# maxrmorrison/torbi

Hardware: AMD Instinct MI355X
Metric: timesteps decoded/sec, 1440 states batch=512 (higher is better)
Workload: dtype f32; 1 GPU; 1440 states, 500 frames, batch=512 per GPU, fp32, dense transition (BASELINE configs[2]); decode = forward + argmax + backtrace, inputs resident in HBM; parallelism=single GPU, streams=2

## Files before the change

### torbi_amd/csrc/lazy_backtrace.hpp

```cpp
#pragma once

#include <hip/hip_runtime.h>
#include <stdint.h>
#include <math.h>

#include "wave_reduce.hpp"

namespace lazy {

constexpr int kSentinel = 0x7fffffff;

__device__ __forceinline__ void take_better(float &v, int &i, float ov, int oi) {
    if (ov > v || (ov == v && oi < i)) { v = ov; i = oi; }
}

__device__ __forceinline__ int wave_first_argmax(float v, int i) {
#pragma unroll
    for (int off = 32; off > 0; off >>= 1) {
        const float ov = __shfl_xor(v, off, 64);
        const int oi = __shfl_xor(i, off, 64);
        take_better(v, i, ov, oi);
    }
    return i;
}

__device__ __forceinline__ void scan1(float c, int i, float &best, int &arg) {
    if (c > best) { best = c; arg = i; }
    else if (arg == kSentinel) { best = c; arg = i; }
}

template <int VEC>
__device__ __forceinline__ void backtrace_item(const float *__restrict__ h, const float *__restrict__ trans, int f,
                                               int32_t *__restrict__ o, int T, int S, int lane) {
    f = f < 1 ? 1 : (f > T ? T : f);

    float best = -INFINITY;
    int arg = kSentinel;
    {
        const float *row = h + (size_t)(f - 1) * S;
        if (VEC == 4) {
            for (int i = 4 * lane; i < S; i += 256) {
                const float4 v = *reinterpret_cast<const float4 *>(row + i);
                scan1(v.x, i, best, arg); scan1(v.y, i + 1, best, arg);
                scan1(v.z, i + 2, best, arg); scan1(v.w, i + 3, best, arg);
            }
        } else {
            for (int i = lane; i < S; i += 64) scan1(row[i], i, best, arg);
        }
    }
    int j = wave_first_argmax(best, arg);

    for (int tt = f - 1 + lane; tt < T; tt += 64) o[tt] = j;

    for (int tt = f - 1; tt >= 1; --tt) {
        const float *row = h + (size_t)(tt - 1) * S;
        const float *tr = trans + (size_t)j * S;
        best = -INFINITY;
        arg = kSentinel;
        if (VEC == 4) {
            for (int i = 4 * lane; i < S; i += 256) {
                const float4 p = *reinterpret_cast<const float4 *>(row + i);
                const float4 q = *reinterpret_cast<const float4 *>(tr + i);
                scan1(p.x + q.x, i, best, arg); scan1(p.y + q.y, i + 1, best, arg);
                scan1(p.z + q.z, i + 2, best, arg); scan1(p.w + q.w, i + 3, best, arg);
            }
        } else {
            for (int i = lane; i < S; i += 64) scan1(row[i] + tr[i], i, best, arg);
        }
        j = wave_first_argmax(best, arg);
        if (lane == 0) o[tt - 1] = j;
    }
}

template <int VEC>
__global__ __launch_bounds__(64) void backtrace_kernel(const float *__restrict__ hist,
                                                       const float *__restrict__ trans,
                                                       const int32_t *__restrict__ frames,
                                                       int32_t *__restrict__ out, int B, int T, int S) {
    const int b = blockIdx.x;
    backtrace_item<VEC>(hist + (size_t)b * T * S, trans, frames[b], out + (size_t)b * T, T, S, threadIdx.x);
}

template <int NQ>
__device__ __forceinline__ int lane_first_equal(const float4 (&v)[NQ], float m, int lane, int S) {
    int k = kSentinel;
#pragma unroll
    for (int q = NQ - 1; q >= 0; --q) {
        const int i = 4 * lane + 256 * q;
        if (i < S) {
            int kq = v[q].w == m ? i + 3 : kSentinel;
            kq = v[q].z == m ? i + 2 : kq;
            kq = v[q].y == m ? i + 1 : kq;
            kq = v[q].x == m ? i : kq;
            k = min(k, kq);
        }
    }
    return k;
}

template <int NQ>
__device__ __forceinline__ float lane_max(const float4 (&v)[NQ], int lane, int S) {
    float m = -INFINITY;
#pragma unroll
    for (int q = 0; q < NQ; ++q)
        if (4 * lane + 256 * q < S)
            m = __builtin_fmaxf(__builtin_fmaxf(m, __builtin_fmaxf(v[q].x, v[q].y)), __builtin_fmaxf(v[q].z, v[q].w));
    return m;
}

template <int NQ>
__device__ __forceinline__ int wave_first_argmax4(const float4 (&v)[NQ], int lane, int S) {
    const float m = wavered::wave_reduce_f32(lane_max<NQ>(v, lane, S), wavered::MaxOp());
    const int k = wavered::wave_min_i32(lane_first_equal<NQ>(v, m, lane, S));
    return k < S ? k : 0;
}

template <int NQ>
__device__ __forceinline__ void backtrace_prefetch_item(const float *__restrict__ h, const float *__restrict__ trans,
                                                        int f, int32_t *__restrict__ o, int T, int S, int lane) {
    f = f < 1 ? 1 : (f > T ? T : f);
    const float4 zero = make_float4(0.f, 0.f, 0.f, 0.f);

    float4 cur[NQ], nxt[NQ];
    {
        const float *row = h + (size_t)(f - 1) * S;
#pragma unroll
        for (int q = 0; q < NQ; ++q) {
            const int i = 4 * lane + 256 * q;
            cur[q] = i < S ? *reinterpret_cast<const float4 *>(row + i) : zero;
        }
    }
    {
        const float *row = h + (size_t)(f >= 2 ? f - 2 : 0) * S;
#pragma unroll
        for (int q = 0; q < NQ; ++q) {
            const int i = 4 * lane + 256 * q;
            nxt[q] = i < S ? *reinterpret_cast<const float4 *>(row + i) : zero;
        }
    }
    int j = wave_first_argmax4<NQ>(cur, lane, S);
    for (int tt = f - 1 + lane; tt < T; tt += 64) o[tt] = j;

    for (int tt = f - 1; tt >= 1; --tt) {
        const float *tr = trans + (size_t)j * S;
        float4 q4[NQ];
#pragma unroll
        for (int q = 0; q < NQ; ++q) {
            const int i = 4 * lane + 256 * q;
            q4[q] = i < S ? *reinterpret_cast<const float4 *>(tr + i) : zero;
        }
#pragma unroll
        for (int q = 0; q < NQ; ++q) cur[q] = nxt[q];
        {
            const float *row = h + (size_t)(tt >= 2 ? tt - 2 : 0) * S;
#pragma unroll
            for (int q = 0; q < NQ; ++q) {
                const int i = 4 * lane + 256 * q;
                nxt[q] = i < S ? *reinterpret_cast<const float4 *>(row + i) : zero;
            }
        }
        float4 cand[NQ];
#pragma unroll
        for (int q = 0; q < NQ; ++q)
            cand[q] = make_float4(cur[q].x + q4[q].x, cur[q].y + q4[q].y, cur[q].z + q4[q].z, cur[q].w + q4[q].w);
        j = wave_first_argmax4<NQ>(cand, lane, S);
        if (lane == 0) o[tt - 1] = j;
    }
}

template <int NQ>
__global__ __launch_bounds__(64) void backtrace_prefetch_kernel(const float *__restrict__ hist,
                                                                const float *__restrict__ trans,
                                                                const int32_t *__restrict__ frames,
                                                                int32_t *__restrict__ out, int B, int T, int S,
                                                                const int32_t *__restrict__ narrow) {
    if (narrow && *narrow <= 512) return;
    const int b = blockIdx.x;
    backtrace_prefetch_item<NQ>(hist + (size_t)b * T * S, trans, frames[b], out + (size_t)b * T, T, S, threadIdx.x);
}

template <int NQ>
struct GatherWalker {
    const float *__restrict__ h;
    const float *__restrict__ rowmax;
    const float2 *__restrict__ sorted;
    int SpP, shift, S, lane;
    __device__ __forceinline__ int first_state(int t) const {
        const float4 zero = make_float4(0.f, 0.f, 0.f, 0.f);
        float4 last[NQ];
        const float *row = h + (size_t)t * S;
#pragma unroll
        for (int q = 0; q < NQ; ++q) {
            const int i = 4 * lane + 256 * q;
            last[q] = i < S ? *reinterpret_cast<const float4 *>(row + i) : zero;
        }
        return wave_first_argmax4<NQ>(last, lane, S);
    }
    __device__ __forceinline__ int step(int j, int tt) const {
        const int Sp = (S + 15) / 16 * 16;
        const float2 *row = sorted + (size_t)j * SpP;
        float2 ent = row[lane];
        const float hmax = rowmax[tt - 1];
        const float *hrow = h + (size_t)(tt - 1) * S;
        float bv = -INFINITY;
        int bi = kSentinel;
        float best = -INFINITY;
        for (int k0 = 0; k0 < Sp; k0 += 64) {
            const int kn = k0 + 64 < SpP ? k0 + 64 : SpP - 1;
            const float tn = row[kn].x;
            if (k0 + lane < Sp) {
                const int i = __float_as_int(ent.y) >> shift;
                const float c = hrow[i] + ent.x;
                if (c > bv || (c == bv && i < bi)) { bv = c; bi = i; }
            }
            best = wavered::wave_reduce_f32(bv, wavered::MaxOp());
            if (k0 + 64 >= Sp || tn + hmax < best) break;
            const int kl = k0 + 64 + lane;
            ent = row[kl < SpP ? kl : SpP - 1];
        }
        const int cand = (bv == best && bi != kSentinel) ? bi : kSentinel;
        const int win = wavered::wave_min_i32(cand);
        return best == -INFINITY ? 0 : win;
    }
};

template <class Walker>
__device__ __forceinline__ int inside(const Walker &w, int j) { return (unsigned)j < (unsigned)w.S ? j : 0; }

template <class Walker>
__device__ __forceinline__ void walk_item(const Walker &w, int f, int32_t *__restrict__ o, int T, int lane) {
    f = f < 1 ? 1 : (f > T ? T : f);
    int j = inside(w, w.first_state(f - 1));
    for (int tt = f - 1 + lane; tt < T; tt += 64) o[tt] = j;
    for (int tt = f - 1; tt >= 1; --tt) {
        j = inside(w, w.step(j, tt));
        if (lane == 0) o[tt - 1] = j;
    }
}

template <class Walker>
__device__ __forceinline__ void chase_segment(const Walker &w, int f, int T, int K, int s, int32_t *__restrict__ o,
                                              int32_t *__restrict__ arrive, int lane) {
    f = f < 1 ? 1 : (f > T ? T : f);
    const int L = (f - 1 + K - 1) / K;
    const int lo = min(s * L, f - 1), hi = min((s + 1) * L, f - 1);
    const bool last = s == K - 1;
    if (!last && lo >= hi) return;
    int j = inside(w, w.first_state(hi));
    if (last) {
        for (int tt = f - 1 + lane; tt < T; tt += 64) o[tt] = j;
    } else if (lane == 0) {
        o[hi] = j;
    }
    for (int tt = hi; tt > lo; --tt) {
        j = inside(w, w.step(j, tt));
        if (lane == 0 && (tt - 1 > lo || s == 0)) o[tt - 1] = j;
    }
    if (lane == 0) arrive[s] = j;
}

template <class Walker>
__device__ __forceinline__ void stitch_segments(const Walker &w, int f, int T, int K, int32_t *__restrict__ o,
                                                const int32_t *__restrict__ arrive, int lane, unsigned *stats = nullptr) {
    f = f < 1 ? 1 : (f > T ? T : f);
    const int L = (f - 1 + K - 1) / K;
    int truth = arrive[K - 1];
    unsigned again = 0;
    for (int s = K - 2; s >= 0; --s) {
        const int lo = min(s * L, f - 1), hi = min((s + 1) * L, f - 1);
        if (lo >= hi) continue;
        if (o[hi] == truth) {
            truth = arrive[s];
            continue;
        }
        int j = truth;
        if (lane == 0) o[hi] = j;
        bool met = false;
        for (int tt = hi; tt > lo; --tt) {
            j = inside(w, w.step(j, tt));
            ++again;
            if (tt - 1 == lo) break;
            if (o[tt - 1] == j) { met = true; break; }
            if (lane == 0) o[tt - 1] = j;
        }
        if (met) {
            truth = arrive[s];
        } else {
            truth = j;
            if (s == 0 && lane == 0) o[0] = j;
        }
    }
    if (stats && lane == 0) {
        atomicAdd(stats, (unsigned)(f - 1));
        atomicAdd(stats + 1, again);
    }
}

template <int NQ>
__device__ __forceinline__ void backtrace_gather_item(const float *__restrict__ h, const float *__restrict__ rowmax,
                                                      const float2 *__restrict__ sorted, int SpP, int shift, int f,
                                                      int32_t *__restrict__ o, int T, int S, int lane) {
    const GatherWalker<NQ> w{h, rowmax, sorted, SpP, shift, S, lane};
    walk_item(w, f, o, T, lane);
}

template <int NQ>
__global__ __launch_bounds__(64) void backtrace_gather_kernel(const float *__restrict__ hist, const float *__restrict__ rowmax,
                                                              const float2 *__restrict__ sorted, int SpP, int shift,
                                                              const int32_t *__restrict__ frames, int32_t *__restrict__ out,
                                                              int B, int T, int S) {
    const int b = blockIdx.x;
    backtrace_gather_item<NQ>(hist + (size_t)b * T * S, rowmax + (size_t)b * T, sorted, SpP, shift, frames[b],
                              out + (size_t)b * T, T, S, threadIdx.x);
}

constexpr int kRangedWindow = 512;

__global__ __launch_bounds__(64) void row_ranges_kernel(const float *__restrict__ trans, int32_t *__restrict__ ranges,
                                                        int32_t *__restrict__ widest, int S) {
    const int j = blockIdx.x, lane = threadIdx.x;
    const float *row = trans + (size_t)j * S;
    int lo = kSentinel, hi = 0;
    for (int i = lane; i < S; i += 64) {
        if (row[i] != -INFINITY) {
            lo = min(lo, i);
            hi = max(hi, i + 1);
        }
    }
    lo = wavered::wave_min_i32(lo);
    hi = -wavered::wave_min_i32(-hi);
    if (lane == 0) {
        if (hi == 0) lo = 0;
        ranges[2 * j] = lo;
        ranges[2 * j + 1] = hi;
        atomicMax(widest, hi - (lo & ~3));
    }
}

template <int NQ>
__global__ __launch_bounds__(64) void backtrace_ranged_kernel(const float *__restrict__ hist, const float *__restrict__ trans,
                                                              const int32_t *__restrict__ ranges,
                                                              const int32_t *__restrict__ widest,
                                                              const int32_t *__restrict__ frames, int32_t *__restrict__ out,
                                                              int B, int T, int S) {
    if (*widest > kRangedWindow) return;
    const int b = blockIdx.x, lane = threadIdx.x;
    const float *h = hist + (size_t)b * T * S;
    int32_t *o = out + (size_t)b * T;
    int f = frames[b];
    f = f < 1 ? 1 : (f > T ? T : f);
    const float4 zero = make_float4(0.f, 0.f, 0.f, 0.f);
    int j;
    {
        float4 last[NQ];
        const float *row = h + (size_t)(f - 1) * S;
#pragma unroll
        for (int q = 0; q < NQ; ++q) {
            const int i = 4 * lane + 256 * q;
            last[q] = i < S ? *reinterpret_cast<const float4 *>(row + i) : zero;
        }
        j = wave_first_argmax4<NQ>(last, lane, S);
    }
    for (int tt = f - 1 + lane; tt < T; tt += 64) o[tt] = j;
    const float4 none = make_float4(-INFINITY, -INFINITY, -INFINITY, -INFINITY);
    for (int tt = f - 1; tt >= 1; --tt) {
        const int lo4 = ranges[2 * j] & ~3, hi = ranges[2 * j + 1];
        const float *tr = trans + (size_t)j * S, *hrow = h + (size_t)(tt - 1) * S;
        float4 cand[2];
#pragma unroll
        for (int q = 0; q < 2; ++q) {
            const int i = lo4 + 4 * lane + 256 * q;
            if (i < hi) {
                const float4 t4 = *reinterpret_cast<const float4 *>(tr + i);
                const float4 p4 = *reinterpret_cast<const float4 *>(hrow + i);
                cand[q] = make_float4(p4.x + t4.x, p4.y + t4.y, p4.z + t4.z, p4.w + t4.w);
            } else {
                cand[q] = none;
            }
        }
        const float m = wavered::wave_reduce_f32(
            __builtin_fmaxf(__builtin_fmaxf(__builtin_fmaxf(cand[0].x, cand[0].y), __builtin_fmaxf(cand[0].z, cand[0].w)),
                            __builtin_fmaxf(__builtin_fmaxf(cand[1].x, cand[1].y), __builtin_fmaxf(cand[1].z, cand[1].w))),
            wavered::MaxOp());
        int k = kSentinel;
#pragma unroll
        for (int q = 1; q >= 0; --q) {
            const int i = lo4 + 4 * lane + 256 * q;
            int kq = cand[q].w == m ? i + 3 : kSentinel;
            kq = cand[q].z == m ? i + 2 : kq;
            kq = cand[q].y == m ? i + 1 : kq;
            kq = cand[q].x == m ? i : kq;
            k = min(k, kq);
        }
        k = wavered::wave_min_i32(k);
        j = (m == -INFINITY || k >= S) ? 0 : k;
        if (lane == 0) o[tt - 1] = j;
    }
}

template <int NQ>
struct RowWalker {
    const float *__restrict__ h;
    const float *__restrict__ trans;
    int S, lane;
    __device__ __forceinline__ int first_state(int t) const {
        const float4 zero = make_float4(0.f, 0.f, 0.f, 0.f);
        float4 last[NQ];
        const float *row = h + (size_t)t * S;
#pragma unroll
        for (int q = 0; q < NQ; ++q) {
            const int i = 4 * lane + 256 * q;
            last[q] = i < S ? *reinterpret_cast<const float4 *>(row + i) : zero;
        }
        return wave_first_argmax4<NQ>(last, lane, S);
    }
    __device__ __forceinline__ int step(int j, int tt) const {
        const float *tr = trans + (size_t)j * S, *hrow = h + (size_t)(tt - 1) * S;
        const float4 zero = make_float4(0.f, 0.f, 0.f, 0.f);
        float4 cand[NQ];
#pragma unroll
        for (int q = 0; q < NQ; ++q) {
            const int i = 4 * lane + 256 * q;
            const float4 t4 = i < S ? *reinterpret_cast<const float4 *>(tr + i) : zero;
            const float4 p4 = i < S ? *reinterpret_cast<const float4 *>(hrow + i) : zero;
            cand[q] = make_float4(p4.x + t4.x, p4.y + t4.y, p4.z + t4.z, p4.w + t4.w);
        }
        return wave_first_argmax4<NQ>(cand, lane, S);
    }
};

template <int NQ>
__global__ __launch_bounds__(64) void segment_rows_kernel(const float *__restrict__ hist, const float *__restrict__ trans,
                                                          const int32_t *__restrict__ frames, int32_t *__restrict__ out, int B,
                                                          int T, int S, int K, int32_t *__restrict__ arrive) {
    const int b = (int)blockIdx.x / K, seg = (int)blockIdx.x - b * K;
    const RowWalker<NQ> w{hist + (size_t)b * T * S, trans, S, (int)threadIdx.x};
    chase_segment(w, frames[b], T, K, seg, out + (size_t)b * T, arrive + (size_t)b * K, threadIdx.x);
}
template <int NQ>
__global__ __launch_bounds__(64) void stitch_rows_kernel(const float *__restrict__ hist, const float *__restrict__ trans,
                                                         const int32_t *__restrict__ frames, int32_t *__restrict__ out, int B,
                                                         int T, int S, int K, const int32_t *__restrict__ arrive) {
    const int b = blockIdx.x;
    const RowWalker<NQ> w{hist + (size_t)b * T * S, trans, S, (int)threadIdx.x};
    stitch_segments(w, frames[b], T, K, out + (size_t)b * T, arrive + (size_t)b * K, threadIdx.x);
}

}
```

### torbi_amd/csrc/pruned_forward.hpp

```cpp
#pragma once

#include <hip/hip_runtime.h>
#include <stdint.h>
#include <math.h>
#include <type_traits>

#include "wave_reduce.hpp"

namespace pruned {

#ifndef TORBI_KR
#define TORBI_KR 3
#endif
constexpr int kR = TORBI_KR;
constexpr int kNB = 16;
constexpr int kBlk = 16;
constexpr int kPad = 4 * kBlk;
constexpr int kTop = kR + 1;
constexpr int kMaxS16 = 2048;
constexpr int kMaxS = 4096;
constexpr int kStatSlots = 64;

__global__ __launch_bounds__(256) void sort_rows_kernel(const float *__restrict__ trans,
                                                        float2 *__restrict__ sorted, int32_t *__restrict__ row_range,
                                                        int S, int SpP, int NPOW, int row_bytes) {
    extern __shared__ float skey[];
    int *sval = reinterpret_cast<int *>(skey + NPOW);
    __shared__ int s_lo, s_hi;
    const int j = blockIdx.x;
    const float *row = trans + (size_t)j * S;
    if (threadIdx.x == 0) { s_lo = S; s_hi = -1; }
    __syncthreads();
    int lo = S, hi = -1;
    for (int k = threadIdx.x; k < NPOW; k += 256) {
        const float v = k < S ? row[k] : -INFINITY;
        skey[k] = v;
        sval[k] = k < S ? k * row_bytes : 0;
        if (v != -INFINITY) { lo = min(lo, k); hi = max(hi, k); }
    }
    if (hi >= 0) { atomicMin(&s_lo, lo); atomicMax(&s_hi, hi); }
    __syncthreads();
    const bool dead = s_hi < 0;
    const int row_lo = dead ? 0 : s_lo, row_hi = dead ? S - 1 : s_hi;
    if (threadIdx.x == 0) { row_range[2 * j] = row_lo; row_range[2 * j + 1] = row_hi; }
    for (int size = 2; size <= NPOW; size <<= 1) {
        for (int stride = size >> 1; stride > 0; stride >>= 1) {
            for (int k = threadIdx.x; k < NPOW; k += 256) {
                const int partner = k ^ stride;
                if (partner > k) {
                    const bool desc = (k & size) == 0;
                    const float a = skey[k], b = skey[partner];
                    if (desc ? (a < b) : (a > b)) {
                        skey[k] = b; skey[partner] = a;
                        const int t = sval[k]; sval[k] = sval[partner]; sval[partner] = t;
                    }
                }
            }
            __syncthreads();
        }
    }
    float2 *out = sorted + (size_t)j * SpP;
    for (int k = threadIdx.x; k < SpP; k += 256) {
        float2 v;
        v.x = k < S ? skey[k] : -INFINITY;
        v.y = __builtin_bit_cast(float, (k < S && v.x != -INFINITY) ? sval[k] : row_lo * row_bytes);
        out[k] = v;
    }
}

template <int RG>
__global__ __launch_bounds__(64) void arrange_blocks_kernel(float2 *__restrict__ sorted, int S, int SpP) {
    constexpr int SHIFT = RG == 4 ? 6 : 5;
    typedef unsigned long long u64;
    const int nblk = SpP / kBlk;
    const int id = blockIdx.x * blockDim.x + threadIdx.x;
    if (id >= (S / RG) * nblk) return;
    const int q = id / nblk, kb = id % nblk;
    u64 present[kBlk];
    {
        const float2 *r0 = sorted + (size_t)(RG * q) * SpP + kb * kBlk;
        for (int p = 0; p < kBlk; ++p) present[p] = (u64)1 << (8 * ((__float_as_int(r0[p].y) >> SHIFT) & (RG - 1)));
    }
    for (int r = 1; r < RG; ++r) {
        float2 *row = sorted + (size_t)(RG * q + r) * SpP + kb * kBlk;
        float2 ent[kBlk], out[kBlk];
        u64 remaining = 0;
        for (int e = 0; e < kBlk; ++e) {
            ent[e] = row[e];
            if (e) remaining += (u64)1 << (8 * ((__float_as_int(ent[e].y) >> SHIFT) & (RG - 1)));
        }
        out[0] = ent[0];
        present[0] += (u64)1 << (8 * ((__float_as_int(ent[0].y) >> SHIFT) & (RG - 1)));
        unsigned used = 1u;
        for (int p = 1; p < kBlk; ++p) {
            int pick = -1, key = 1 << 30;
            for (int e = 1; e < kBlk; ++e) {
                if ((used >> e) & 1u) continue;
                const int res = (__float_as_int(ent[e].y) >> SHIFT) & (RG - 1);
                const int k = (int)((present[p] >> (8 * res)) & 0xffu) * 64 - (int)((remaining >> (8 * res)) & 0xffu);
                if (k < key) { key = k; pick = e; }
            }
            const int res = (__float_as_int(ent[pick].y) >> SHIFT) & (RG - 1);
            used |= 1u << pick;
            remaining -= (u64)1 << (8 * res);
            present[p] += (u64)1 << (8 * res);
            out[p] = ent[pick];
        }
        for (int p = 1; p < kBlk; ++p) row[p] = out[p];
    }
}

__global__ __launch_bounds__(256) void transpose_kernel(const float *__restrict__ trans, float *__restrict__ tt,
                                                        int S) {
    __shared__ float tile[32][33];
    const int x0 = blockIdx.x * 32, y0 = blockIdx.y * 32;
    const int tx = threadIdx.x & 31, ty = threadIdx.x >> 5;
    for (int r = ty; r < 32; r += 8)
        tile[r][tx] = (y0 + r < S && x0 + tx < S) ? trans[(size_t)(y0 + r) * S + x0 + tx] : 0.f;
    __syncthreads();
    for (int r = ty; r < 32; r += 8)
        if (x0 + r < S && y0 + tx < S) tt[(size_t)(x0 + r) * S + y0 + tx] = tile[tx][r];
}

__global__ __launch_bounds__(256) void init_history_kernel(const float *__restrict__ obs,
                                                           const float *__restrict__ initial,
                                                           float *__restrict__ hist, int B, int T, int S) {
    const size_t n = (size_t)B * S;
    for (size_t e = (size_t)blockIdx.x * blockDim.x + threadIdx.x; e < n;
         e += (size_t)gridDim.x * blockDim.x) {
        const int b = (int)(e / S);
        const int i = (int)(e - (size_t)b * S);
        hist[(size_t)b * T * S + i] = obs[(size_t)b * T * S + i] + initial[i];
    }
}


template <int EPL>
struct ListBlock { float4 e[EPL / 2]; };

template <int EPL>
__device__ __forceinline__ void load_list_block(ListBlock<EPL> &blk, const float2 *row_g, int k) {
#pragma unroll
    for (int h = 0; h < EPL / 2; ++h) blk.e[h] = *reinterpret_cast<const float4 *>(row_g + k + 2 * h);
}

template <int G, int O>
__device__ __forceinline__ int group_bcast(int x) {
    constexpr int ctrl = G == 4 ? O * 0x55 : (O | (O << 2) | ((2 + O) << 4) | ((2 + O) << 6));
    return __builtin_amdgcn_update_dpp(0, x, ctrl, 0xf, 0xf, true);
}
template <int G, int O>
__device__ __forceinline__ float group_bcast(float x) {
    return __builtin_bit_cast(float, group_bcast<G, O>(__builtin_bit_cast(int, x)));
}

}
```

### torbi_amd/csrc/resident_forward.hpp

```cpp
#pragma once

#include <hip/hip_runtime.h>
#include <stdint.h>
#include <math.h>
#include <type_traits>

#include "pruned_forward.hpp"
#include "lazy_backtrace.hpp"
#include "nonfinite.hpp"

namespace resident {

using pruned::kBlk;
using pruned::kR;
using pruned::kTop;
using pruned::ListBlock;
using pruned::group_bcast;
using pruned::load_list_block;

constexpr int kNI = 16;
constexpr int kMaxBatches = 16;
constexpr int kRowGroup = 16;
#ifndef TORBI_TILE16_MAX_S
#define TORBI_TILE16_MAX_S pruned::kMaxS16
#endif
__host__ __device__ inline int tile_items(int S) { return S <= TORBI_TILE16_MAX_S ? kNI : kNI / 2; }
__host__ __device__ inline int pass_rows(int S) { return 64 / (tile_items(S) / 4); }

typedef unsigned long long u64;

struct Batch {
    const float *obs;
    const int32_t *frames;
    float *hist;
    int32_t *out;
    const int32_t *order;
    float *rowmax;
    int B, T;
    int tile0;
    int item0;
    int32_t *alarm;
};

struct Group {
    Batch batch[kMaxBatches];
    int n;
    const int32_t *tile_map;
    unsigned *stats;
    const unsigned *only;
    int serial;
};

#ifndef RESIDENT_MAX_R
#define RESIDENT_MAX_R 16
#endif
constexpr int kMaxR = RESIDENT_MAX_R;
constexpr int kMaxTop = 4;
constexpr unsigned kAbsentBits = 0x7fd5a5a5u;
constexpr int kSlots = 4;
__host__ __device__ inline size_t cluster_slot_bytes(int S) {
    return ((size_t)S + 3) / 4 * 4 * kNI * sizeof(float) +
           (size_t)kMaxR * kNI * kMaxTop * 2 * sizeof(u64);
}
struct Cluster {
    float *xchg;
    unsigned *where;
    int tiles;
    unsigned *control;
    unsigned *failed;
    int R;
    unsigned long long wait_ticks;
    int spread;
};
constexpr unsigned long long kClusterWaitTicks = 25000000ull;

inline bool supported(int S) { return S >= 64 && S <= pruned::kMaxS; }

inline size_t lds_bytes(int S, int ktop = kTop) {
    const size_t S4 = ((size_t)S + 3) / 4 * 4, ni = (size_t)tile_items(S);
    return sizeof(float) * ni * S4 + sizeof(u64) * kNI * ktop + (sizeof(float) + sizeof(int)) * kNI * ktop +
           2 * sizeof(int) * kNI + 4 * sizeof(int);
}

__host__ __device__ inline int cluster_first_group(int m, int nrg, int R) { return (int)((long long)m * nrg / R); }

constexpr int kMaxOrdered = 8192;
struct OrderJob { const int32_t *frames; int32_t *order; int B, T, tile0; int32_t *hist; int32_t *route_record; int route; };
struct OrderJobs { OrderJob job[kMaxBatches]; int ascending; int n; int tiles; int32_t *tile_map; unsigned *stats;
                   unsigned *flags; int nflags;
                   int ni; };

__global__ __launch_bounds__(256) void order_items_kernel(OrderJobs jobs) {
    const OrderJob &jb = jobs.job[blockIdx.y];
    const int b = blockIdx.x * 256 + threadIdx.x;
    const int B = jb.B, T = jb.T;
    if (b == 0 && jb.route_record) *jb.route_record = jb.route;
    if (b >= B) return;
    if (B > kMaxOrdered) return;
    int f = jb.frames[b];
    f = f < 1 ? 1 : (f > T ? T : f);
    int rank = 0;
    for (int o = 0; o < B; ++o) {
        int g = jb.frames[o];
        g = g < 1 ? 1 : (g > T ? T : g);
        rank += (g > f) || (g == f && o < b);
    }
    jb.order[jobs.ascending ? B - 1 - rank : rank] = b;
}

__global__ __launch_bounds__(256) void order_large_count_kernel(OrderJob jb) {
    const int b = blockIdx.x * 256 + threadIdx.x;
    if (b >= jb.B) return;
    int f = jb.frames[b];
    f = f < 1 ? 1 : (f > jb.T ? jb.T : f);
    atomicAdd(&jb.hist[f], 1);
}

__global__ __launch_bounds__(1024) void order_large_scan_kernel(OrderJob jb, int ascending) {
    __shared__ int part[1024];
    const int T = jb.T, tid = threadIdx.x;
    const int per = (T + 1024) / 1024;
    auto length_at = [&](int k) { return ascending ? 1 + k : T - k; };
    int sum = 0;
    for (int k = tid * per; k < (tid + 1) * per && k < T; ++k) sum += jb.hist[length_at(k)];
    part[tid] = sum;
    __syncthreads();
    if (tid == 0) {
        int run = 0;
        for (int i = 0; i < 1024; ++i) { const int v = part[i]; part[i] = run; run += v; }
    }
    __syncthreads();
    int run = part[tid];
    for (int k = tid * per; k < (tid + 1) * per && k < T; ++k) {
        const int f = length_at(k), v = jb.hist[f];
        jb.hist[f] = run;
        run += v;
    }
}

__global__ __launch_bounds__(256) void order_large_place_kernel(OrderJob jb) {
    const int b = blockIdx.x * 256 + threadIdx.x;
    if (b >= jb.B) return;
    int f = jb.frames[b];
    f = f < 1 ? 1 : (f > jb.T ? jb.T : f);
    jb.order[atomicAdd(&jb.hist[f], 1)] = b;
}

__global__ __launch_bounds__(256) void order_tiles_kernel(OrderJobs jobs) {
    const int w = blockIdx.x * 256 + threadIdx.x;
    if (w < 128) jobs.stats[w] = 0u;
    for (int k = w; k < jobs.nflags; k += gridDim.x * 256) jobs.flags[k] = 0u;
    if (w >= jobs.tiles) return;
    auto tile_length = [&](int k, int j) {
        const OrderJob &jb = jobs.job[k];
        const int last = jobs.ni * j + jobs.ni - 1 < jb.B ? jobs.ni * j + jobs.ni - 1 : jb.B - 1;
        int f = jb.frames[jb.order[jobs.ascending ? last : jobs.ni * j]];
        return f < 1 ? 1 : (f > jb.T ? jb.T : f);
    };
    int k = 0;
    for (int q = 1; q < jobs.n; ++q)
        if (w >= jobs.job[q].tile0) k = q;
    const int j = w - jobs.job[k].tile0;
    const int mine = tile_length(k, j);
    int rank = 0;
    for (int q = 0; q < jobs.n; ++q) {
        const int nt = (jobs.job[q].B + jobs.ni - 1) / jobs.ni;
        for (int t = 0; t < nt; ++t) {
            const int other = tile_length(q, t);
            const int ow = jobs.job[q].tile0 + t;
            rank += (other > mine) || (other == mine && ow < w);
        }
    }
    jobs.tile_map[jobs.ascending ? jobs.tiles - 1 - rank : rank] = (k << 20) | j;
}

__global__ __launch_bounds__(256) void absent_kernel(uint4 *__restrict__ slots, size_t granules) {
    const uint4 a = {kAbsentBits, kAbsentBits, kAbsentBits, kAbsentBits};
    for (size_t g = (size_t)blockIdx.x * 256 + threadIdx.x; g < granules; g += (size_t)gridDim.x * 256) slots[g] = a;
}

__device__ __forceinline__ u64 top_key(float v, int state) {
    unsigned u = __float_as_uint(v);
    u ^= (u >> 31) ? 0xffffffffu : 0x80000000u;
    return ((u64)u << 32) | (unsigned)(0x7fffffff - state);
}

template <int KTOP = kTop>
__device__ __forceinline__ void top_insert(u64 *list, u64 x) {
    if (x <= list[KTOP - 1]) return;
#pragma unroll
    for (int r = 0; r < KTOP; ++r) {
        if (x != 0ull) {
            const u64 old = atomicMax(&list[r], x);
            x = old < x ? old : (old == x ? 0ull : x);
        }
    }
}

typedef unsigned int v4u __attribute__((ext_vector_type(4)));
__device__ __forceinline__ void store_through(__amdgpu_buffer_rsrc_t buffer, int offset, float4 v) {
    v4u x = {__float_as_uint(v.x), __float_as_uint(v.y), __float_as_uint(v.z), __float_as_uint(v.w)};
    __builtin_amdgcn_raw_buffer_store_b128(x, buffer, offset, 0, 16);
}
__device__ __forceinline__ void store_plain(__amdgpu_buffer_rsrc_t buffer, int offset, float4 v) {
    v4u x = {__float_as_uint(v.x), __float_as_uint(v.y), __float_as_uint(v.z), __float_as_uint(v.w)};
    __builtin_amdgcn_raw_buffer_store_b128(x, buffer, offset, 0, 0);
}
__device__ __forceinline__ float4 load_through(__amdgpu_buffer_rsrc_t buffer, int offset) {
    const v4u x = __builtin_amdgcn_raw_buffer_load_b128(buffer, offset, 0, 16);
    return make_float4(__uint_as_float(x.x), __uint_as_float(x.y), __uint_as_float(x.z), __uint_as_float(x.w));
}
__device__ __forceinline__ __amdgpu_buffer_rsrc_t buffer_of(const void *base, unsigned bytes) {
    return __builtin_amdgcn_make_buffer_rsrc(const_cast<void *>(base), 0, (int)bytes, 0x00020000);
}

#ifndef RESIDENT_ABL
#define RESIDENT_ABL 0
#endif
#ifndef CLUSTER_POLL_SLEEP
#define CLUSTER_POLL_SLEEP 4
#endif
#ifndef CLUSTER_ROUND
#define CLUSTER_ROUND 8
#endif
#ifndef RESIDENT_EXTRA_VALU
#define RESIDENT_EXTRA_VALU 0
#endif

#ifdef RESIDENT_STAMP
constexpr int kPhases = 12;
__device__ unsigned long long g_phase[1024 * 16 * kPhases];
__device__ unsigned long long g_wgtime[1024 * 4];
#define RSTAMP(i) { const unsigned long long now_ = __builtin_readcyclecounter(); acc[i] += now_ - last; last = now_; }
#define RCOUNT(i, n) acc[i] += (n)
#else
#define RSTAMP(i)
#define RCOUNT(i, n)
#endif

template <int KW, int MAXP, bool PIPE, int KR = kR, bool CLUSTER = false, int NI = 16, bool REPAIR = false>
__global__ __launch_bounds__(64 * KW) void resident_forward_kernel(Group grp, Cluster clu, const float *__restrict__ tt,
                                                                   const float2 *__restrict__ sorted,
                                                                   const float *__restrict__ initial, int S, int SpP) {
    constexpr int kNI = NI, G = NI / 4, EPL = kBlk / G, kRowGroup = 64 / G;
    constexpr int kR = KR, kTop = KR + 1;
    static_assert(NI == 16 || NI == 8, "tiles of 16 or 8 items");
    extern __shared__ __attribute__((aligned(16))) float lds[];
    const int S4 = (S + 3) / 4 * 4;
    u64 *top = reinterpret_cast<u64 *>(lds + (size_t)kNI * S4);
    float *mtopv = reinterpret_cast<float *>(top + kNI * kTop);
    int *mtopi = reinterpret_cast<int *>(mtopv + kNI * kTop);
    int *sframes = mtopi + kNI * kTop;
    int *sitem = sframes + kNI;
    int *smisc = sitem + kNI;

    const int tid = threadIdx.x, lane = tid & 63;
    const int wave = __builtin_amdgcn_readfirstlane(tid >> 6);
    const unsigned long long clock_0 = clock64(), wall_0 = wall_clock64();
#ifdef RESIDENT_STAMP
    const unsigned long long wg_start = wall_clock64();
#endif

    int cid = blockIdx.x, member = 0;
    const int R = CLUSTER ? clu.R : 1;
    if constexpr (REPAIR) {
        if (!grp.only || grp.only[blockIdx.x] == 0u) return;
    }
    bool local = false;
    if constexpr (CLUSTER) {
        const int cls = blockIdx.x & 7;
        if (tid == 0) {
            smisc[0] = (int)__hip_atomic_fetch_add(clu.control + cls, 1u, __ATOMIC_RELAXED, __HIP_MEMORY_SCOPE_AGENT);
            smisc[1] = 0;
        }
        __syncthreads();
        const int ticket = __builtin_amdgcn_readfirstlane(smisc[0]);
        if (clu.spread) {
            const int per = R / 8;
            member = cls * per + ticket % per;
            cid = ticket / per;
        } else {
            member = ticket % R;
            cid = (ticket / R) * 8 + cls;
        }
        if (cid >= clu.tiles) return;
        if (wave == 0) {
            unsigned *const where = clu.where + (size_t)cid * kMaxR;
            const unsigned xcc = __builtin_amdgcn_s_getreg(20 | (0 << 6) | (3 << 11)) & 15u;
            if (lane == 0) __hip_atomic_store(where + member, xcc + 1u, __ATOMIC_RELAXED, __HIP_MEMORY_SCOPE_AGENT);
            unsigned long long since = 0ull;
            unsigned seen = xcc + 1u;
            bool complete = true;
            for (;;) {
                if (lane < R) seen = __hip_atomic_load(where + lane, __ATOMIC_RELAXED, __HIP_MEMORY_SCOPE_AGENT);
                if (__all(seen != 0u)) break;
                const unsigned long long now = wall_clock64();
                if (since == 0ull) since = now;
                if (now - since >= clu.wait_ticks) { complete = false; break; }
                __builtin_amdgcn_s_sleep(8);
            }
            const bool same = complete && __all(seen == xcc + 1u);
            if (lane == 0) smisc[2] = same ? 1 : 0;
        }
        __syncthreads();
#ifndef CLUSTER_LOCAL_EXCHANGE
#define CLUSTER_LOCAL_EXCHANGE 1
#endif
        local = CLUSTER_LOCAL_EXCHANGE && smisc[2] != 0;
    }
    const int code = grp.tile_map[cid];
    const Batch &bat = grp.batch[code >> 20];
    const float *__restrict__ obs = bat.obs;
    float *__restrict__ hist = bat.hist;
    const int B = bat.B, T = bat.T;
    const int b0 = (code & 0xfffff) * kNI;
    bool odd = false;

    if (tid < kNI) {
        int f = 0;
        const int item = bat.order[b0 + tid < B ? b0 + tid : B - 1];
        if (b0 + tid < B) {
            f = bat.frames[item];
            f = f < 1 ? 1 : (f > T ? T : f);
        }
        sframes[tid] = f;
        sitem[tid] = item;
    }
    if (tid < kNI * kTop) top[tid] = 0ull;
    __syncthreads();
    int fmax = 0;
#pragma unroll
    for (int it = 0; it < kNI; ++it) fmax = max(fmax, sframes[it]);

    for (int item = 0; item < kNI; ++item) {
        const int b = sitem[item];
        const bool valid = b0 + item < B;
        const float *src = obs + (size_t)b * T * S;
        float *dst = hist + (size_t)b * T * S;
        for (int i = tid; i < S; i += 64 * KW) {
            const float v = src[i] + initial[i];
            odd = odd || nonfinite::odd(v);
            lds[i * kNI + item] = v;
            if (valid) dst[i] = v;
            top_insert<kTop>(top + item * kTop, top_key(v, i));
        }
    }

    const int g = lane & (G - 1);
    const int jl = G == 4 ? (int)((0xFBAE9DC873261540ull >> (4 * (lane >> 2))) & 15)
                          : (int)((0xFE7654DC32BA9810ull >> (4 * ((lane >> 1) & 15))) & 15) + (lane & 32) / 2;
    const char *ptile = reinterpret_cast<const char *>(lds) + 16 * g;
    const int nrg = (S + kRowGroup - 1) / kRowGroup;
    const int rg_lo = CLUSTER ? cluster_first_group(member, nrg, R) : 0;
    const int rg_hi = CLUSTER ? cluster_first_group(member + 1, nrg, R) : nrg;
    const unsigned xrow = (unsigned)S4 * kNI * (unsigned)sizeof(float);
    const unsigned xbytes = (unsigned)cluster_slot_bytes(S);
    static_assert(kTop <= kMaxTop, "a member publishes at most kMaxTop list entries per item");
    int ib[4];
#pragma unroll
    for (int it = 0; it < 4; ++it) ib[it] = sitem[4 * g + it];

    float pend[MAXP][4];
    const int own_lo = kRowGroup * rg_lo, own_hi = kRowGroup * rg_hi < S ? kRowGroup * rg_hi : S;
    const int pieces = CLUSTER ? (S - (own_hi - own_lo)) * G : 0;
    auto place = [&](int c) {
        int row = c / G;
        row = row < own_lo ? row : row + (own_hi - own_lo);
        return (row * kNI + 4 * (c % G)) * 4;
    };
#ifndef RESIDENT_FIXED8
#define RESIDENT_FIXED8 1
#endif
#ifndef RESIDENT_FIXED16
#define RESIDENT_FIXED16 1
#endif
    constexpr bool FIXED = CLUSTER && MAXP == 1 && (NI == 16 ? RESIDENT_FIXED16 : RESIDENT_FIXED8);
    ListBlock<EPL> head0, head1;
    float obnext[4] = {0.f, 0.f, 0.f, 0.f};
    if constexpr (FIXED) {
        const int rg = rg_lo + wave;
        const int jj = kRowGroup * rg + jl;
        const int jr = (rg < rg_hi && jj < S) ? jj : S - 1;
        const float2 *row = sorted + (size_t)jr * SpP + EPL * g;
        load_list_block(head0, row, 0);
        load_list_block(head1, row, kBlk);
        if (fmax > 1) {
#pragma unroll
            for (int it = 0; it < 4; ++it) obnext[it] = obs[((size_t)ib[it] * T + 1) * S + jr];
        }
    }
    unsigned stat_blocks = 0, stat_passes = 0;

    auto publish_top = [&](int row) {
        if (tid < kNI * kTop) {
            const u64 key = top[tid];
            unsigned u = (unsigned)(key >> 32);
            u ^= (u >> 31) ? 0x80000000u : 0xffffffffu;
            const float value = key ? __uint_as_float(u) : -INFINITY;
            mtopv[tid] = value;
            mtopi[tid] = key ? (0x7fffffff - (int)(unsigned)key) * S : 0;
            top[tid] = 0ull;
            const int item = tid / kTop;
            if (tid == item * kTop && member == 0 && b0 + item < B && row < sframes[item])
                bat.rowmax[(size_t)sitem[item] * T + row] = value;
        }
    };
    __syncthreads();
    publish_top(0);
#ifdef RESIDENT_STAMP
    unsigned long long acc[kPhases] = {};
    unsigned long long last = __builtin_readcyclecounter();
#endif

    for (int t = 1; t < fmax; ++t) {
        __syncthreads();
        RSTAMP(0);

        float seedv[4][kR ? kR : 1], thr[4];
        int seedo[4][kR ? kR : 1];
        bool live[4];
#pragma unroll
        for (int it = 0; it < 4; ++it) {
            const int item = 4 * g + it;
            live[it] = t < sframes[item];
            if constexpr (kTop == 4) {
                const float4 v = *reinterpret_cast<const float4 *>(mtopv + item * kTop);
                const int4 o = *reinterpret_cast<const int4 *>(mtopi + item * kTop);
                const float vv[4] = {v.x, v.y, v.z, v.w};
                const int oo[4] = {o.x, o.y, o.z, o.w};
#pragma unroll
                for (int r = 0; r < kR; ++r) { seedv[it][r] = vv[r]; seedo[it][r] = oo[r]; }
                thr[it] = live[it] ? vv[kR] : -INFINITY;
            } else {
#pragma unroll
                for (int r = 0; r < kR; ++r) { seedv[it][r] = mtopv[item * kTop + r]; seedo[it][r] = mtopi[item * kTop + r]; }
                thr[it] = live[it] ? mtopv[item * kTop + kR] : -INFINITY;
            }
        }
        RSTAMP(1);

        int opaque = 0;
        asm volatile("" : "+s"(opaque));
#pragma unroll
        for (int p = 0; p < MAXP; ++p) {
            const int rg = rg_lo + wave + KW * p + opaque;
            if (rg < rg_hi) {
                const int jj = kRowGroup * rg + jl;
                const bool jv = jj < S;
                const int jr = jv ? jj : S - 1;
                const float2 *row = sorted + (size_t)jr * SpP + EPL * g;
                ListBlock<EPL> cur, nxt;
                float ob[4];
                if constexpr (FIXED) {
                    cur = head0;
                    nxt = head1;
#pragma unroll
                    for (int it = 0; it < 4; ++it) ob[it] = obnext[it];
                } else {
                    load_list_block(cur, row, 0);
                    load_list_block(nxt, row, kBlk);
#pragma unroll
                    for (int it = 0; it < 4; ++it)
                        ob[it] = (RESIDENT_ABL & 32) ? 0.5f * it : obs[((size_t)ib[it] * T + t) * S + jr];
                }
                float seedt[4][kR ? kR : 1];
#pragma unroll
                for (int it = 0; it < 4; ++it)
#pragma unroll
                    for (int r = 0; r < kR; ++r)
                        seedt[it][r] = (RESIDENT_ABL & 64) ? -1.0f : tt[(unsigned)(seedo[it][r] + jr)];

                float best[4] = {-INFINITY, -INFINITY, -INFINITY, -INFINITY};
#if RESIDENT_EXTRA_VALU
                float dummy[4] = {0.f, 0.f, 0.f, 0.f};
#endif
                struct PairData { float4 p0, p1; float t0, t1; };
// ... 327 lines not shown
```

Baseline: 55.69 million timesteps/s.

## Cut register pressure in helper kernels and stage ranking data in shared memory

Rewrites the backtrace first-state argmax as a rolled strided loop followed by wave reductions, replacing the fully unrolled float4 array. Moves the arrange_blocks per-thread entry and present arrays into shared memory with 4-bit packed counters and vectorized loads, writing each output row entry as soon as it is picked. Order_items and order_tiles now load frame/tile lengths in chunks into shared memory and rank against them with int4 reads instead of each thread rereading global memory. The aim is lower register use and less global traffic in these setup and backtrace kernels. The risks are extra __syncthreads, the packed 4-bit counters overflowing if a residue count exceeds 15, and the rolled loops losing ILP.

```diff
diff --git a/torbi_amd/csrc/lazy_backtrace.hpp b/torbi_amd/csrc/lazy_backtrace.hpp
--- a/torbi_amd/csrc/lazy_backtrace.hpp
+++ b/torbi_amd/csrc/lazy_backtrace.hpp
@@ -186,15 +186,20 @@
     const float2 *__restrict__ sorted;
     int SpP, shift, S, lane;
     __device__ __forceinline__ int first_state(int t) const {
-        const float4 zero = make_float4(0.f, 0.f, 0.f, 0.f);
-        float4 last[NQ];
         const float *row = h + (size_t)t * S;
-#pragma unroll
-        for (int q = 0; q < NQ; ++q) {
-            const int i = 4 * lane + 256 * q;
-            last[q] = i < S ? *reinterpret_cast<const float4 *>(row + i) : zero;
-        }
-        return wave_first_argmax4<NQ>(last, lane, S);
+        float bv = -INFINITY;
+        int bi = kSentinel;
+#pragma unroll 1
+        for (int i = 4 * lane; i < S; i += 256) {
+            const float4 v = *reinterpret_cast<const float4 *>(row + i);
+            if (v.x > bv || (v.x == bv && i < bi)) { bv = v.x; bi = i; }
+            if (v.y > bv || (v.y == bv && i + 1 < bi)) { bv = v.y; bi = i + 1; }
+            if (v.z > bv || (v.z == bv && i + 2 < bi)) { bv = v.z; bi = i + 2; }
+            if (v.w > bv || (v.w == bv && i + 3 < bi)) { bv = v.w; bi = i + 3; }
+        }
+        const float m = wavered::wave_reduce_f32(bv, wavered::MaxOp());
+        const int k = wavered::wave_min_i32(bv == m ? bi : kSentinel);
+        return k < S ? k : 0;
     }
     __device__ __forceinline__ int step(int j, int tt) const {
         const int Sp = (S + 15) / 16 * 16;
diff --git a/torbi_amd/csrc/pruned_forward.hpp b/torbi_amd/csrc/pruned_forward.hpp
--- a/torbi_amd/csrc/pruned_forward.hpp
+++ b/torbi_amd/csrc/pruned_forward.hpp
@@ -72,41 +72,52 @@
 __global__ __launch_bounds__(64) void arrange_blocks_kernel(float2 *__restrict__ sorted, int S, int SpP) {
     constexpr int SHIFT = RG == 4 ? 6 : 5;
     typedef unsigned long long u64;
+    __shared__ float2 s_ent[kBlk][64];
+    __shared__ unsigned s_present[kBlk][64];
     const int nblk = SpP / kBlk;
-    const int id = blockIdx.x * blockDim.x + threadIdx.x;
+    const int tid = threadIdx.x;
+    const int id = blockIdx.x * blockDim.x + tid;
     if (id >= (S / RG) * nblk) return;
     const int q = id / nblk, kb = id % nblk;
-    u64 present[kBlk];
     {
         const float2 *r0 = sorted + (size_t)(RG * q) * SpP + kb * kBlk;
-        for (int p = 0; p < kBlk; ++p) present[p] = (u64)1 << (8 * ((__float_as_int(r0[p].y) >> SHIFT) & (RG - 1)));
+#pragma unroll 2
+        for (int p = 0; p < kBlk; ++p) s_present[p][tid] = 1u << (4 * ((__float_as_int(r0[p].y) >> SHIFT) & (RG - 1)));
     }
+#pragma unroll 1
     for (int r = 1; r < RG; ++r) {
         float2 *row = sorted + (size_t)(RG * q + r) * SpP + kb * kBlk;
-        float2 ent[kBlk], out[kBlk];
-        u64 remaining = 0;
-        for (int e = 0; e < kBlk; ++e) {
-            ent[e] = row[e];
-            if (e) remaining += (u64)1 << (8 * ((__float_as_int(ent[e].y) >> SHIFT) & (RG - 1)));
+        u64 residue = 0;
+        unsigned remaining = 0;
+#pragma unroll 2
+        for (int e = 0; e < kBlk; e += 2) {
+            const float4 v = *reinterpret_cast<const float4 *>(row + e);
+            s_ent[e][tid] = make_float2(v.x, v.y);
+            s_ent[e + 1][tid] = make_float2(v.z, v.w);
+            const int r0 = (__float_as_int(v.y) >> SHIFT) & (RG - 1), r1 = (__float_as_int(v.w) >> SHIFT) & (RG - 1);
+            residue |= ((u64)r0 << (4 * e)) | ((u64)r1 << (4 * e + 4));
+            if (e) remaining += 1u << (4 * r0);
+            remaining += 1u << (4 * r1);
         }
-        out[0] = ent[0];
-        present[0] += (u64)1 << (8 * ((__float_as_int(ent[0].y) >> SHIFT) & (RG - 1)));
+        s_present[0][tid] += 1u << (4 * (int)(residue & 15u));
         unsigned used = 1u;
+#pragma unroll 1
         for (int p = 1; p < kBlk; ++p) {
+            const unsigned present = s_present[p][tid];
             int pick = -1, key = 1 << 30;
+#pragma unroll 1
             for (int e = 1; e < kBlk; ++e) {
                 if ((used >> e) & 1u) continue;
-                const int res = (__float_as_int(ent[e].y) >> SHIFT) & (RG - 1);
-                const int k = (int)((present[p] >> (8 * res)) & 0xffu) * 64 - (int)((remaining >> (8 * res)) & 0xffu);
+                const int res = (int)(residue >> (4 * e)) & 15;
+                const int k = (int)((present >> (4 * res)) & 15u) * 64 - (int)((remaining >> (4 * res)) & 15u);
                 if (k < key) { key = k; pick = e; }
             }
-            const int res = (__float_as_int(ent[pick].y) >> SHIFT) & (RG - 1);
+            const int res = (int)(residue >> (4 * pick)) & 15;
             used |= 1u << pick;
-            remaining -= (u64)1 << (8 * res);
-            present[p] += (u64)1 << (8 * res);
-            out[p] = ent[pick];
+            remaining -= 1u << (4 * res);
+            s_present[p][tid] = present + (1u << (4 * res));
+            row[p] = s_ent[pick][tid];
         }
-        for (int p = 1; p < kBlk; ++p) row[p] = out[p];
     }
 }
 
diff --git a/torbi_amd/csrc/resident_forward.hpp b/torbi_amd/csrc/resident_forward.hpp
--- a/torbi_amd/csrc/resident_forward.hpp
+++ b/torbi_amd/csrc/resident_forward.hpp
@@ -90,22 +90,35 @@
                    unsigned *flags; int nflags;
                    int ni; };
 
+constexpr int kOrderChunk = 2048;
 __global__ __launch_bounds__(256) void order_items_kernel(OrderJobs jobs) {
+    __shared__ __align__(16) int s_len[kOrderChunk];
     const OrderJob &jb = jobs.job[blockIdx.y];
     const int b = blockIdx.x * 256 + threadIdx.x;
     const int B = jb.B, T = jb.T;
     if (b == 0 && jb.route_record) *jb.route_record = jb.route;
-    if (b >= B) return;
+    if ((int)blockIdx.x * 256 >= B) return;
     if (B > kMaxOrdered) return;
-    int f = jb.frames[b];
+    int f = b < B ? jb.frames[b] : 1;
     f = f < 1 ? 1 : (f > T ? T : f);
     int rank = 0;
-    for (int o = 0; o < B; ++o) {
-        int g = jb.frames[o];
-        g = g < 1 ? 1 : (g > T ? T : g);
-        rank += (g > f) || (g == f && o < b);
-    }
-    jb.order[jobs.ascending ? B - 1 - rank : rank] = b;
+    for (int o0 = 0; o0 < B; o0 += kOrderChunk) {
+        const int n = min(kOrderChunk, B - o0), n4 = (n + 3) / 4 * 4;
+        if (o0) __syncthreads();
+        for (int o = threadIdx.x; o < n4; o += 256) {
+            int g = o < n ? jb.frames[o0 + o] : 0;
+            s_len[o] = o < n ? (g < 1 ? 1 : (g > T ? T : g)) : 0;
+        }
+        __syncthreads();
+        for (int o = 0; o < n4; o += 4) {
+            const int4 g = *reinterpret_cast<const int4 *>(&s_len[o]);
+            rank += (g.x > f) || (g.x == f && o0 + o < b);
+            rank += (g.y > f) || (g.y == f && o0 + o + 1 < b);
+            rank += (g.z > f) || (g.z == f && o0 + o + 2 < b);
+            rank += (g.w > f) || (g.w == f && o0 + o + 3 < b);
+        }
+    }
+    if (b < B) jb.order[jobs.ascending ? B - 1 - rank : rank] = b;
 }
 
 __global__ __launch_bounds__(256) void order_large_count_kernel(OrderJob jb) {
@@ -147,31 +160,45 @@
 }
 
 __global__ __launch_bounds__(256) void order_tiles_kernel(OrderJobs jobs) {
+    __shared__ __align__(16) int s_len[kOrderChunk];
     const int w = blockIdx.x * 256 + threadIdx.x;
     if (w < 128) jobs.stats[w] = 0u;
     for (int k = w; k < jobs.nflags; k += gridDim.x * 256) jobs.flags[k] = 0u;
-    if (w >= jobs.tiles) return;
+    if ((int)blockIdx.x * 256 >= jobs.tiles) return;
+    auto batch_of_tile = [&](int v) {
+        int k = 0;
+        for (int q = 1; q < jobs.n; ++q)
+            if (v >= jobs.job[q].tile0) k = q;
+        return k;
+    };
     auto tile_length = [&](int k, int j) {
         const OrderJob &jb = jobs.job[k];
         const int last = jobs.ni * j + jobs.ni - 1 < jb.B ? jobs.ni * j + jobs.ni - 1 : jb.B - 1;
         int f = jb.frames[jb.order[jobs.ascending ? last : jobs.ni * j]];
         return f < 1 ? 1 : (f > jb.T ? jb.T : f);
     };
-    int k = 0;
-    for (int q = 1; q < jobs.n; ++q)
-        if (w >= jobs.job[q].tile0) k = q;
+    const bool live = w < jobs.tiles;
+    const int k = live ? batch_of_tile(w) : 0;
     const int j = w - jobs.job[k].tile0;
-    const int mine = tile_length(k, j);
+    const int mine = live ? tile_length(k, j) : 1;
     int rank = 0;
-    for (int q = 0; q < jobs.n; ++q) {
-        const int nt = (jobs.job[q].B + jobs.ni - 1) / jobs.ni;
-        for (int t = 0; t < nt; ++t) {
-            const int other = tile_length(q, t);
-            const int ow = jobs.job[q].tile0 + t;
-            rank += (other > mine) || (other == mine && ow < w);
-        }
-    }
-    jobs.tile_map[jobs.ascending ? jobs.tiles - 1 - rank : rank] = (k << 20) | j;
+    for (int v0 = 0; v0 < jobs.tiles; v0 += kOrderChunk) {
+        const int n = min(kOrderChunk, jobs.tiles - v0), n4 = (n + 3) / 4 * 4;
+        if (v0) __syncthreads();
+        for (int v = threadIdx.x; v < n4; v += 256) {
+            const int kv = v < n ? batch_of_tile(v0 + v) : 0;
+            s_len[v] = v < n ? tile_length(kv, v0 + v - jobs.job[kv].tile0) : 0;
+        }
+        __syncthreads();
+        for (int v = 0; v < n4; v += 4) {
+            const int4 g = *reinterpret_cast<const int4 *>(&s_len[v]);
+            rank += (g.x > mine) || (g.x == mine && v0 + v < w);
+            rank += (g.y > mine) || (g.y == mine && v0 + v + 1 < w);
+            rank += (g.z > mine) || (g.z == mine && v0 + v + 2 < w);
+            rank += (g.w > mine) || (g.w == mine && v0 + v + 3 < w);
+        }
+    }
+    if (live) jobs.tile_map[jobs.ascending ? jobs.tiles - 1 - rank : rank] = (k << 20) | j;
 }
 
 __global__ __launch_bounds__(256) void absent_kernel(uint4 *__restrict__ slots, size_t granules) {
```

Result: faster. 57.20 million timesteps/s (median of 6 runs) (+2.7%).
